# AshuiRUA/NPI-GNN

Hardware: AMD Instinct MI355X
Metric: edges/sec per GNN layer (fwd+bwd) (higher is better)
Workload: dtype f32; 1 GPU; C4 synthetic ncRNA-protein bipartite graph, N=1000000 nodes, E=20000000 directed edges (both directions, Zipf-skewed protein side), 1 SAGEConv layer 256->256 fp32, fwd+bwd incl. dX/dW/db, graph+features resident in HBM; parallelism=single GPU, hip_graph_replay=False, setup_steps=40, csr_sorted_columns=True

## Files before the change

### include/npi_gnn.h

```cpp
#ifndef NPI_GNN_H
#define NPI_GNN_H

#include <stdint.h>

#ifdef __cplusplus
extern "C" {
#endif

#define NPI_OK 0
#define NPI_ERR_ARG (-1)
#define NPI_ERR_LAUNCH (-2)
#define NPI_ERR_WORKSPACE (-3)

#ifndef NPI_ITEM_EDGES
#define NPI_ITEM_EDGES 256
#endif

#define NPI_F32 0
#define NPI_BF16 1

const char* npi_last_error(void);
int npi_abi_version(void);

int64_t npi_csr_workspace_bytes(int64_t E, int64_t N);
int64_t npi_item_edges(int64_t nnz_max);
int64_t npi_num_items(int64_t nnz_max, int64_t item_edges);

#define NPI_CSR_DROP_EQUAL 1
#define NPI_CSR_SORT_COLUMNS 2
int npi_csr_build_ex(const int64_t* key_nodes, const int64_t* val_nodes, int64_t E, int64_t N,
                     int64_t n_cols, int add_self_loops, int64_t loop_col_offset, int build_flags,
                     int32_t* rowptr, int32_t* col, int32_t* eid, int32_t* rowidx,
                     int32_t* item_row, int64_t item_edges, int32_t* status,
                     void* workspace, int64_t workspace_bytes, void* stream);

int npi_edge_positions(const int32_t* eid, const int32_t* rowptr, int64_t N, int64_t nnz_max,
                       int64_t E, int32_t* pos_of, void* stream);

int64_t npi_segsum_carry_elems(int64_t nnz_max, int64_t item_edges, int64_t F);
int npi_segsum_scales_supported(int64_t F, int dtype);
int npi_segsum_ex(const int32_t* rowptr, const int32_t* col, const int32_t* item_row, int64_t item_edges,
                   const float* w, int64_t N, int64_t nnz_max, const void* x, int64_t ldx,
                   const void* x2, int64_t split, void* out, int64_t ldo, int64_t F, int dtype, int mean,
                   const float* bias, float* carry, float* row_scales_out, void* stream);

#define NPI_HUB_MAX 128
int64_t npi_hub_plan_workspace_elems(void);
int npi_hub_plan(const int32_t* rowptr, const int32_t* col, int64_t N, int64_t n_cols, int64_t nnz_max, int64_t h_max,
                 int64_t min_degree, int64_t min_entries, int32_t* hub_rows, uint32_t* mask, int32_t* info, int32_t* workspace,
                 void* stream);
int npi_hub_light_side(const int32_t* rowptr, const int32_t* col, const int32_t* eid, const int32_t* rowidx, int64_t N,
                       int64_t nnz_max, const int32_t* hub_rows, int64_t H, int64_t nnz_max_light, int64_t item_edges,
                       int32_t* rowptr_l, int32_t* col_l, int32_t* eid_l, int32_t* rowidx_l, int32_t* item_row_l, void* stream);
int64_t npi_segsum_hub_slabs(int64_t n_cols);
int64_t npi_segsum_hub_partial_elems(int64_t n_cols);
int npi_segsum_hub(const int32_t* hub_rows, int64_t H, const uint32_t* mask, const int32_t* rowptr, int64_t N, int64_t n_cols,
                   const float* col_scale, const float* x, int64_t ldx, float* out, int64_t ldo, int64_t F, int mean,
                   float* partial, float* row_scales_out, void* stream);

int npi_row_weight_sum(const int32_t* rowptr, const float* w, int64_t N, float* deg, void* stream);
int npi_gcn_norm(const int32_t* rowidx, const int32_t* col, const int32_t* rowptr, const float* w,
                 const float* deg, const int32_t* deg_rowptr, int64_t N, int64_t nnz_max, float* norm,
                 void* stream);
int npi_entry_col_scale(const int32_t* col, const int32_t* rowptr, const float* table, const float* w_in, int64_t N, int64_t n_cols,
                        int64_t nnz_max, float* w_out, void* stream);
int npi_row_inv_count(const int32_t* rowptr, int64_t N, float* inv_cnt, void* stream);
int npi_entry_weights(const int32_t* eid, const int32_t* rowidx, const int32_t* rowptr,
                      const float* edge_w, const float* loop_w_node, float fill,
                      int64_t N, int64_t nnz_max, float* w_entry, void* stream);
int npi_edge_dot(const int32_t* rowptr, const int32_t* col, const int32_t* rowidx, const int32_t* eid, int64_t N, int64_t n_cols,
                 int64_t nnz_max, int64_t n_edges, const float* a, int64_t lda, const float* b, int64_t ldb, int64_t F,
                 const float* row_scale, const float* mul, float* g_entry, float* gm_entry, float* d_edge, float* d_loop,
                 void* stream);
int npi_gcn_norm_bwd(const int32_t* rowptr, const int32_t* col, const int32_t* rowidx, const int32_t* eid, int64_t N,
                     int64_t nnz_max, int64_t n_edges, const float* g_entry, const float* deg, const float* s_a, const float* s_b,
                     float* d_edge, float* d_loop, void* stream);
int npi_hold_cus(int workgroups, int64_t nanoseconds, uint64_t* start_word, void* stream);
int npi_relu_backward(const float* dy, int64_t ldd, const float* y, int64_t ldy, int64_t M, int64_t F, float* dz, int64_t ldz,
                      void* stream);

#define NPI_STATUS_BAD_ROW_ID 8
int npi_rows_gather(const void* x, int64_t ldx, int64_t n_src, const int64_t* idx, int64_t n, int64_t F, void* out, int64_t ldo,
                    int dtype, int32_t* status, void* stream);

int npi_l2_normalize_rows(const float* x, int64_t ldx, int64_t M, int64_t F, float eps, float* y, int64_t ldy, float* norm,
                          void* stream);
int npi_l2_normalize_rows_bwd(const float* dy, int64_t ldd, const float* y, int64_t ldy, const float* norm, int64_t M, int64_t F,
                              float eps, float* dx, int64_t ldx, void* stream);


int64_t npi_colsum_workspace_elems(int64_t M, int64_t N);
int npi_colsum(const float* X, int64_t ldx, int64_t M, int64_t N, float* out, float* workspace,
               int64_t workspace_elems, void* stream);
int64_t npi_linear_bwd_weight_workspace_elems(int64_t M, int64_t K, int64_t N);

#define NPI_GEMM_EXACT_F32 1
#define NPI_GEMM_SPLIT_BF16 2
#define NPI_GEMM_A_ZERO_PADDED 4
#define NPI_GEMM_WORKSPACE_PREPARED 8
#define NPI_GEMM_RESERVE_CUS(n) ((((n) / 8) & 0xff) << 8)
#define NPI_GEMM_RESERVED_CUS_OF(flags) ((((flags) >> 8) & 0xff) * 8)
#define NPI_GEMM_SPLIT_F16X2 16
#define NPI_PREPARE_F16X2 4
int64_t npi_linear_workspace_bytes(int64_t K, int64_t N);
int npi_row_scales(const float* A, int64_t lda, int64_t M, int64_t K, float* scales, void* stream);
int npi_linear_prepare(const void* W, int64_t ldw, int64_t K, int64_t N, int which, int dtype, void* workspace,
                       int64_t workspace_bytes, void* stream);
int npi_linear_bwd_weight_ex(const void* A, int64_t lda, const void* dC, int64_t lddc,
                             void* dW, int64_t lddw, void* db,
                             int64_t M, int64_t K, int64_t N,
                             float* workspace, int64_t workspace_elems, int dtype, int flags, int shared,
                             const float* a_col_scales, const float* dc_col_scales, void* stream);
int64_t npi_col_scales_workspace_elems(int64_t M, int64_t K);
int npi_col_scales(const float* A, int64_t lda, int64_t M, int64_t K, const float* row_scales, float* scales,
                   float* workspace, int64_t workspace_elems, void* stream);
int npi_linear_fwd_ex(const void* A, int64_t lda, const void* W, int64_t ldw, const void* bias,
                       const float* rowscale, void* C, int64_t ldc,
                       int64_t M, int64_t K, int64_t N, int relu, int dtype, int flags,
                       void* workspace, int64_t workspace_bytes, const float* a_scales, void* stream);
int npi_linear_bwd_data_ex(const void* dC, int64_t lddc, const void* W, int64_t ldw,
                            const float* rowscale, void* dA, int64_t ldda,
                            int64_t M, int64_t K, int64_t N, int dtype, int flags,
                            void* workspace, int64_t workspace_bytes, const float* dc_scales, void* stream);

int npi_linear_fwd_scores_supported(int64_t M, int64_t K, int64_t N);
int npi_linear_fwd_scores(const float* A, int64_t lda, const float* W, int64_t ldw, const float* att, float* C, int64_t ldc,
                              float* sc0, float* sc1, int64_t M, int64_t K, int64_t N, void* workspace, int64_t workspace_bytes,
                              const float* a_scales, void* stream);
int npi_linear_bwd_data_rank2_supported(int64_t M, int64_t K, int64_t N);
int npi_linear_bwd_data_rank2(const float* dC, int64_t lddc, const float* W, int64_t ldw, const float* row0,
                                  const float* row1, const float* col0, const float* col1, float* dA, int64_t ldda,
                                  int64_t M, int64_t K, int64_t N, void* workspace, int64_t workspace_bytes,
                                  const float* dc_scales, void* stream);

int npi_gat_rank2_cols(const float* W, int64_t ldw, const float* att, int64_t K, int64_t C, float* U, void* stream);
int npi_gat_rank2_tail(const float* P, const float* W, int64_t ldw, const float* att, int64_t K, int64_t C, float* dw, int64_t lddw,
                       float* datt, void* stream);

int npi_conv_fwd(const int32_t* rowptr, const int32_t* col, const int32_t* item_row, int64_t item_edges,
                 const float* w_entry, int64_t N, int64_t nnz_max, const void* x, int64_t ldx, int64_t F, int mean,
                 void* agg, int64_t ldagg, float* carry, const void* W, int64_t ldw, const void* bias, void* out,
// ... 153 lines not shown
```

### npi_gnn_amd/_lib.py

```python
from __future__ import annotations

import ctypes
import os
from ctypes import c_char_p, c_float, c_int, c_int64, c_void_p

import torch

HERE = os.path.dirname(os.path.abspath(__file__))
LIB_PATH = os.environ.get("NPI_GNN_LIB") or os.path.join(HERE, "libnpi_gnn.so")

NPI_F32 = 0
NPI_BF16 = 1
NPI_GEMM_EXACT_F32 = 1
NPI_GEMM_SPLIT_BF16 = 2
NPI_GEMM_A_ZERO_PADDED = 4
NPI_GEMM_WORKSPACE_PREPARED = 8
NPI_GEMM_SPLIT_F16X2 = 16
NPI_PREPARE_F16X2 = 4
NPI_STATUS_BAD_ROW_ID = 8
NPI_STATUS_BAD_TARGET_ID = 16
NPI_STATUS_BAD_SAMPLE_SIZES = 32
NPI_HUB_MAX = 128


def NPI_GEMM_RESERVE_CUS(n: int) -> int:
    n = int(n)
    if n < 0 or n > 128 or n % 8:
        raise ValueError(f"NPI_GEMM_RESERVE_CUS: a multiple of 8 in [0, 128], got {n}")
    return (n // 8) << 8

_P = c_void_p
_I = c_int64

PROTOTYPES = {
    "npi_last_error": (c_char_p, []),
    "npi_abi_version": (c_int, []),
    "npi_csr_workspace_bytes": (_I, [_I, _I]),
    "npi_item_edges": (_I, [_I]),
    "npi_num_items": (_I, [_I, _I]),
    "npi_csr_build_ex": (c_int, [_P, _P, _I, _I, _I, c_int, _I, c_int, _P, _P, _P, _P, _P, _I, _P, _P, _I, _P]),
    "npi_edge_positions": (c_int, [_P, _P, _I, _I, _I, _P, _P]),
    "npi_segsum_carry_elems": (_I, [_I, _I, _I]),
    "npi_segsum_ex": (c_int, [_P, _P, _P, _I, _P, _I, _I, _P, _I, _P, _I, _P, _I, _I, c_int, c_int, _P, _P, _P, _P]),
    "npi_segsum_scales_supported": (c_int, [_I, c_int]),
    "npi_hub_plan_workspace_elems": (_I, []),
    "npi_hub_plan": (c_int, [_P, _P, _I, _I, _I, _I, _I, _I, _P, _P, _P, _P, _P]),
    "npi_hub_light_side": (c_int, [_P, _P, _P, _P, _I, _I, _P, _I, _I, _I, _P, _P, _P, _P, _P, _P]),
    "npi_segsum_hub_slabs": (_I, [_I]),
    "npi_segsum_hub_partial_elems": (_I, [_I]),
    "npi_segsum_hub": (c_int, [_P, _I, _P, _P, _I, _I, _P, _P, _I, _P, _I, _I, c_int, _P, _P, _P]),
    "npi_row_weight_sum": (c_int, [_P, _P, _I, _P, _P]),
    "npi_gcn_norm": (c_int, [_P, _P, _P, _P, _P, _P, _I, _I, _P, _P]),
    "npi_row_inv_count": (c_int, [_P, _I, _P, _P]),
    "npi_entry_col_scale": (c_int, [_P, _P, _P, _P, _I, _I, _I, _P, _P]),
    "npi_entry_weights": (c_int, [_P, _P, _P, _P, _P, c_float, _I, _I, _P, _P]),
    "npi_edge_dot": (c_int, [_P, _P, _P, _P, _I, _I, _I, _I, _P, _I, _P, _I, _I, _P, _P, _P, _P, _P, _P, _P]),
    "npi_gcn_norm_bwd": (c_int, [_P, _P, _P, _P, _I, _I, _I, _P, _P, _P, _P, _P, _P, _P]),
    "npi_relu_backward": (c_int, [_P, _I, _P, _I, _I, _I, _P, _I, _P]),
    "npi_rows_gather": (c_int, [_P, _I, _I, _P, _I, _I, _P, _I, c_int, _P, _P]),
    "npi_l2_normalize_rows": (c_int, [_P, _I, _I, _I, c_float, _P, _I, _P, _P]),
    "npi_l2_normalize_rows_bwd": (c_int, [_P, _I, _P, _I, _P, _I, _I, c_float, _P, _I, _P]),
    "npi_colsum_workspace_elems": (_I, [_I, _I]),
    "npi_colsum": (c_int, [_P, _I, _I, _I, _P, _P, _I, _P]),
    "npi_linear_bwd_weight_workspace_elems": (_I, [_I, _I, _I]),
    "npi_linear_workspace_bytes": (_I, [_I, _I]),
    "npi_row_scales": (c_int, [_P, _I, _I, _I, _P, _P]),
    "npi_linear_fwd_ex": (c_int, [_P, _I, _P, _I, _P, _P, _P, _I, _I, _I, _I, c_int, c_int, c_int, _P, _I, _P, _P]),
    "npi_linear_bwd_data_ex": (c_int, [_P, _I, _P, _I, _P, _P, _I, _I, _I, _I, c_int, c_int, _P, _I, _P, _P]),
    "npi_linear_prepare": (c_int, [_P, _I, _I, _I, c_int, c_int, _P, _I, _P]),
    "npi_hold_cus": (c_int, [c_int, _I, _P, _P]),
    "npi_linear_fwd_scores_supported": (c_int, [_I, _I, _I]),
    "npi_linear_fwd_scores": (c_int, [_P, _I, _P, _I, _P, _P, _I, _P, _P, _I, _I, _I, _P, _I, _P, _P]),
    "npi_linear_bwd_data_rank2_supported": (c_int, [_I, _I, _I]),
    "npi_linear_bwd_data_rank2": (c_int, [_P, _I, _P, _I, _P, _P, _P, _P, _P, _I, _I, _I, _I, _P, _I, _P, _P]),
    "npi_gat_rank2_cols": (c_int, [_P, _I, _P, _I, _I, _P, _P]),
    "npi_gat_rank2_tail": (c_int, [_P, _P, _I, _P, _I, _I, _P, _I, _P, _P]),
    "npi_linear_bwd_weight_ex": (c_int, [_P, _I, _P, _I, _P, _I, _P, _I, _I, _I, _P, _I, c_int, c_int, c_int, _P, _P, _P]),
    "npi_col_scales_workspace_elems": (_I, [_I, _I]),
    "npi_col_scales": (c_int, [_P, _I, _I, _I, _P, _P, _P, _I, _P]),
    "npi_conv_fwd": (c_int, [_P, _P, _P, _I, _P, _I, _I, _P, _I, _I, c_int, _P, _I, _P, _P, _I, _P, _P, _I, _I, _I, c_int, c_int, c_int,
                             c_int, _P, _I, _P]),
    "npi_conv_bwd": (c_int, [_P, _I, _P, _I, _P, _I, _I, _I, _I, c_int, c_int, _P, _I, _P, _I, _P, _P, _I, _P, _I, _P, _P, _I, _P, _I,
                             c_int, _P, _P, _P, _I, _P, _I, _P, _I, _P, _P]),
    "npi_gat_aggregate_fused": (c_int, [_P, _P, _P, _P, _I, _I, _I, _P, _I, _P, _I, _P, _I, _I, _P, _P, c_float, _P, c_int, _P, _P, _P, _P,
                                            _P]),
    "npi_gat_scores": (c_int, [_P, _I, _P, _I, _I, _I, _P, _P, _P]),
    "npi_gat_aggregate_ex": (c_int, [_P, _P, _P, _I, _I, _I, _P, _I, _P, _I, _P, _I, _I, _I, _P, _P, _P, _P, c_float, c_int,
                                     _P, _P, _P, _P, _P, _P, _P, _P]),
    "npi_gat_pack_targets": (c_int, [_P, _P, _P, _P, _I, _P, _P]),
    "npi_gat_backward_fused_heads": (c_int, [_P, _P, _P, _P, _I, _I, _I, _P, _I, _P, _I, _P, _I, _P, _I, _I, _I, _P, _P, c_float, _P,
                                                 _P, _P, _P, _P, _I, _P]),
    "npi_gat_rank1_add": (c_int, [_P, _I, _P, _P, _P, _I, _I, _I, _P]),
    "npi_gat_rowdot": (c_int, [_P, _I, _P, _I, _P, _I, _I, _I, _P, _P]),
    "npi_gat_edge_grad_ex": (c_int, [_P, _P, _P, _I, _I, _P, _I, _P, _I, _P, _I, _I, _I, _P, _P, _P, _P, _P, c_float,
                                     c_int, _P, _P, _P]),
    "npi_seg_scan_workspace_elems": (_I, [_I, _I]),
    "npi_seg_rowsum_ex": (c_int, [_P, _P, _P, _P, _I, _I, _I, _P, _P, _I, _P]),
    "npi_gat_softmax_stats_ex": (c_int, [_P, _P, _P, _P, _P, _I, _I, _I, c_float, _P, _P, _P, _P, _I, _P]),
    "npi_gat_aggregate_scores": (c_int, [_P, _P, _P, _I, _I, _I, _P, _I, _P, _I, _P, _I, _I, _P, _P, _P, _P, c_int, _P, _P]),
    "npi_gat_rowdot_colsum_workspace_elems": (_I, [_I, _I, _I]),
    "npi_gat_rowdot_colsum_relu": (c_int, [_P, _I, _P, _I, _P, _I, _I, _I, _P, _P, _P, _I, _P, _I, _P]),
    "npi_entry_transpose_map": (c_int, [_P, _P, _P, _P, _P, _I, _I, _P, _P]),
    "npi_gat_att_grad_workspace_elems": (_I, [_I, _I, _I]),
    "npi_gat_att_grad": (c_int, [_P, _I, _P, _P, _I, _I, _I, _P, _P, _I, _P]),
    "npi_topk_score": (c_int, [_P, _I, _P, _I, _I, _P, _P]),
    "npi_graph_bounds": (c_int, [_P, _I, _I, _P, _P]),
    "npi_topk_select": (c_int, [_P, _P, _I, _I, c_float, _P, _P, _P, _P, _I, _P]),
    "npi_topk_sorted_workspace_bytes": (_I, [_I]),
    "npi_topk_select_sorted": (c_int, [_P, _P, _P, _I, _I, c_float, _P, _P, _P, _P, _I, _P]),
    "npi_topk_gather": (c_int, [_P, _I, _P, _P, _P, _P, _I, _I, _I, _P, _I, _P, _P, _P, _P]),
    "npi_filter_adj_workspace_elems": (_I, [_I]),
    "npi_filter_adj": (c_int, [_P, _P, _I, _P, _P, _P, _P, _P, c_int, _P]),
    "npi_filter_adj_newpos_offset": (_I, [_I]),
    "npi_csr_filter_max_rows": (_I, []),
    "npi_csr_filter_workspace_elems": (_I, [_I]),
    "npi_csr_filter": (c_int, [_P, _P, _P, _P, _P, _P, _I, _I, _P, _P, _P, _P, _P, _I, _P, _P, _P]),
    "npi_readout_max_mean": (c_int, [_P, _I, _P, _I, _I, _P, _P]),
    "npi_topk_gather_bwd": (c_int, [_P, _I, _P, _P, _P, _I, _I, _P, _I, _P, _P, _I, _P, _P, _P]),
    "npi_topk_gather_bwd_ex": (c_int, [_P, _I, _P, _P, _P, _I, _I, _P, _I, _P, _P, _I, _P, _P, _P]),
    "npi_topk_weight_grad_workspace_elems": (_I, [_I, _I]),
    "npi_topk_weight_grad": (c_int, [_P, _I, _P, _P, _P, _I, _I, _P, _P, _P, _I, _P]),
    "npi_readout_max_mean_bwd": (c_int, [_P, _I, _P, _I, _I, _P, _P, _P, _I, _P]),
    "npi_readout_max_mean_bwd_ex": (c_int, [_P, _I, _P, _I, _I, _P, _P, _P, _I, _I, _P]),
    "npi_confusion_update": (c_int, [_P, _I, _I, _P, _I, _P, _P]),
    "npi_mlp_head_fwd": (c_int, [_P, _I, _P, _I, _P, _I, _I, _I, _P, _P, _I, _P, _P, _I, _P, _P, _I, _P, c_float, c_int,
                                 _P, _P, _P, _P, _P]),
    "npi_mlp_head_workspace_elems": (_I, [_I, _I, _I, _I]),
    "npi_mlp_head_bwd": (c_int, [_I, _I, _I, _I, _I, _P, _P, _P, _P, c_float, c_int, _P, _P, _P, _P, _P, _P, _P, _P, _P, _P, _P, _P,
                                 _P, _I, _P]),
    "npi_subgraph_sizes": (c_int, [_P, _P, _P, _P, _I, _P, _P, _P, _P]),
    "npi_subgraph_fill": (c_int, [_P, _P, _P, _P, _I, _P, _P, _P, _P, _P, _P, _I, _I, _P, _P]),
    "npi_subgraph_features": (c_int, [_P, _I, _I, _P, _P, _P, _I, _I, _P, _I, _P]),
    "npi_sample_counts": (c_int, [_P, _I, _P, _I, _I, c_float, _P, _P, _P]),
# ... 67 lines not shown
```

### npi_gnn_amd/csrc/segsum_hub.hip

```cpp
#include "npi_common.h"

namespace npi {

constexpr int HUB_WAVES = 8;
constexpr int HUB_PER_WAVE = NPI_HUB_MAX / HUB_WAVES;
constexpr int HUB_THREADS = HUB_WAVES * WAVE;
constexpr int HUB_TILE = 32;
constexpr int HUB_TILE_LOADS = HUB_TILE / HUB_WAVES;
constexpr int HUB_SLAB = 2048;
constexpr int HUB_F = 256;
constexpr int HUB_MASK_WORDS = NPI_HUB_MAX / 32;
constexpr int FIN_WAVES = 16;
static_assert(HUB_PER_WAVE == 16 && HUB_MASK_WORDS == 4, "the wave's 16 mask bits are cut out of four 32-bit words");
static_assert(HUB_TILE == 32 && HUB_TILE % HUB_WAVES == 0, "one mask row per lane of a half wave");

__device__ __forceinline__ uint32_t wave_pattern(const uint4& m, int w) {
    return ((m.x >> w) & 0x01010101u) | (((m.y >> w) & 0x01010101u) << 1) | (((m.z >> w) & 0x01010101u) << 2) |
           (((m.w >> w) & 0x01010101u) << 3);
}
constexpr uint32_t pattern_bit(int k) { return 1u << (8 * (k & 3) + (k >> 2)); }
__device__ __forceinline__ int hub_of(int k, int w) { return ((k >> 2) * 32) + (k & 3) * 8 + w; }

__device__ __forceinline__ void hub_prefetch(const float* __restrict__ x, int64_t ldx, const uint4* __restrict__ mask,
                                             const float* __restrict__ col_scale, int t0, int r1, int w, int lane,
                                             float4 (&pre)[HUB_TILE_LOADS], uint32_t& pat_n, uint32_t& need_n, float& cs_n) {
    const int row = t0 + lane;
    const bool valid = lane < HUB_TILE && row < r1;
    uint4 m = make_uint4(0u, 0u, 0u, 0u);
    if (valid) m = mask[row];
    cs_n = (valid && col_scale != nullptr) ? col_scale[row] : 1.f;
    pat_n = wave_pattern(m, w);
    need_n = (uint32_t)__ballot((m.x | m.y | m.z | m.w) != 0u);
#pragma unroll
    for (int t = 0; t < HUB_TILE_LOADS; ++t) {
        const int i = w + HUB_WAVES * t;
        if ((need_n >> i) & 1u)
            pre[t] = *reinterpret_cast<const float4*>(x + (int64_t)(t0 + i) * ldx + lane * 4);
    }
}

__global__ void __launch_bounds__(HUB_THREADS, 4)
hub_stream_kernel(const float* __restrict__ x, int64_t ldx, const uint4* __restrict__ mask, const float* __restrict__ col_scale,
                  int n_cols, int H, float* __restrict__ partial) {
    __shared__ float4 tile[HUB_TILE][WAVE];
    const int lane = lane_id();
    const int w = uniform_i(threadIdx.x >> 6);
    const int r0 = blockIdx.x * HUB_SLAB;
    const int r1 = min(r0 + HUB_SLAB, n_cols);

    float4 acc[HUB_PER_WAVE];
#pragma unroll
    for (int k = 0; k < HUB_PER_WAVE; ++k) acc[k] = make_float4(0.f, 0.f, 0.f, 0.f);

    float4 pre[HUB_TILE_LOADS];
#pragma unroll
    for (int t = 0; t < HUB_TILE_LOADS; ++t) pre[t] = make_float4(0.f, 0.f, 0.f, 0.f);
    uint32_t pat_n = 0, need_n = 0;
    float cs_n = 1.f;
    if (r0 < r1) hub_prefetch(x, ldx, mask, col_scale, r0, r1, w, lane, pre, pat_n, need_n, cs_n);
    for (int t0 = r0; t0 < r1; t0 += HUB_TILE) {
        __syncthreads();
#pragma unroll
        for (int t = 0; t < HUB_TILE_LOADS; ++t) {
            const int i = w + HUB_WAVES * t;
            if ((need_n >> i) & 1u) tile[i][lane] = pre[t];
        }
        const uint32_t pat = pat_n;
        const float cs = cs_n;
        __syncthreads();
        if (t0 + HUB_TILE < r1) hub_prefetch(x, ldx, mask, col_scale, t0 + HUB_TILE, r1, w, lane, pre, pat_n, need_n, cs_n);
#pragma unroll
        for (int k = 0; k < HUB_PER_WAVE; ++k) {
            uint32_t m = (uint32_t)__ballot((pat & pattern_bit(k)) != 0u);
            while (m != 0u) {
                const int i = uniform_i(__builtin_ctz(m));
                m &= m - 1u;
                const float s = bcast_f(cs, i);
                const float4 v = tile[i][lane];
                acc[k].x = fmaf(v.x, s, acc[k].x);
                acc[k].y = fmaf(v.y, s, acc[k].y);
                acc[k].z = fmaf(v.z, s, acc[k].z);
                acc[k].w = fmaf(v.w, s, acc[k].w);
            }
        }
    }
    float4* __restrict__ dst = reinterpret_cast<float4*>(partial) + (int64_t)blockIdx.x * NPI_HUB_MAX * WAVE;
#pragma unroll
    for (int k = 0; k < HUB_PER_WAVE; ++k) {
        const int j = hub_of(k, w);
        if (j < H) dst[(int64_t)j * WAVE + lane] = acc[k];
    }
}

__device__ __forceinline__ float4 add4(const float4& a, const float4& b) { return make_float4(a.x + b.x, a.y + b.y, a.z + b.z, a.w + b.w); }

__global__ void __launch_bounds__(FIN_WAVES * WAVE)
hub_finish_kernel(const float* __restrict__ partial, int n_slabs, const int32_t* __restrict__ hub_rows, const int32_t* __restrict__ rowptr,
                  int mean, float* __restrict__ out, int64_t ldo, float* __restrict__ scale_out) {
    __shared__ float4 part[FIN_WAVES][WAVE];
    const int lane = lane_id();
    const int w = uniform_i(threadIdx.x >> 6);
    const int j = blockIdx.x;
    const int chunk = (n_slabs + FIN_WAVES - 1) / FIN_WAVES;
    const int s0 = w * chunk, s1 = min(s0 + chunk, n_slabs);
    const float4* __restrict__ src = reinterpret_cast<const float4*>(partial) + (int64_t)j * WAVE + lane;
    const int64_t step = (int64_t)NPI_HUB_MAX * WAVE;
    float4 a = make_float4(0.f, 0.f, 0.f, 0.f);
    int s = s0;
    for (; s + 8 <= s1; s += 8) {
        float4 v[8];
#pragma unroll
        for (int u = 0; u < 8; ++u) v[u] = src[(int64_t)(s + u) * step];
#pragma unroll
        for (int u = 0; u < 8; ++u) a = add4(a, v[u]);
    }
    for (; s < s1; ++s) a = add4(a, src[(int64_t)s * step]);
    part[w][lane] = a;
    __syncthreads();
    if (w != 0) return;
    a = part[0][lane];
#pragma unroll
    for (int g = 1; g < FIN_WAVES; ++g) a = add4(a, part[g][lane]);
    const int r = hub_rows[j];
    float sc = 1.f;
    if (mean) sc = 1.f / (float)max(rowptr[r + 1] - rowptr[r], 1);
    const float4 t = make_float4(fmaf(a.x, sc, 0.f), fmaf(a.y, sc, 0.f), fmaf(a.z, sc, 0.f), fmaf(a.w, sc, 0.f));
    *reinterpret_cast<float4*>(out + (int64_t)r * ldo + lane * 4) = t;
    if (scale_out != nullptr) {
        float m = fmaxf(fmaxf(fabsf(t.x), fabsf(t.y)), fmaxf(fabsf(t.z), fabsf(t.w)));
#pragma unroll
        for (int o = 32; o >= 1; o >>= 1) m = fmaxf(m, __shfl_xor(m, o));
        if (lane == 0) scale_out[r] = pow2_scale_of(m);
    }
}

}

using namespace npi;

extern "C" int64_t npi_segsum_hub_slabs(int64_t n_cols) { return n_cols <= 0 ? 0 : ceil_div(n_cols, HUB_SLAB); }

extern "C" int64_t npi_segsum_hub_partial_elems(int64_t n_cols) {
    return n_cols < 0 ? -1 : (npi_segsum_hub_slabs(n_cols) > 0 ? npi_segsum_hub_slabs(n_cols) : 1) * NPI_HUB_MAX * HUB_F;
}

extern "C" int npi_segsum_hub(const int32_t* hub_rows, int64_t H, const uint32_t* mask, const int32_t* rowptr, int64_t N, int64_t n_cols,
                              const float* col_scale, const float* x, int64_t ldx, float* out, int64_t ldo, int64_t F, int mean,
                              float* partial, float* row_scales_out, void* stream_) {
    hipStream_t stream = (hipStream_t)stream_;
    NPI_REQUIRE(H >= 0 && H <= NPI_HUB_MAX, "npi_segsum_hub: H must be in [0, NPI_HUB_MAX]");
    NPI_REQUIRE(F == HUB_F, "npi_segsum_hub: f32 rows of 256 columns only");
    NPI_REQUIRE(N >= 0 && n_cols >= 0 && n_cols < ((int64_t)1 << 31) - HUB_SLAB, "npi_segsum_hub: bad size");
    if (H == 0) return NPI_OK;
    NPI_REQUIRE(hub_rows && mask && rowptr && x && out && partial, "npi_segsum_hub: null pointer");
    NPI_REQUIRE(ldx >= F && ldo >= F && ldx % 4 == 0 && ldo % 4 == 0 && ((uintptr_t)x % 16) == 0 && ((uintptr_t)out % 16) == 0 &&
                    ((uintptr_t)partial % 16) == 0 && ((uintptr_t)mask % 16) == 0,
                "npi_segsum_hub: rows and masks must be 16-byte aligned");
    const int64_t n_slabs = npi_segsum_hub_slabs(n_cols);
    if (n_slabs > 0) {
        hipLaunchKernelGGL(hub_stream_kernel, dim3((unsigned)n_slabs), dim3(HUB_THREADS), 0, stream, x, ldx,
                           reinterpret_cast<const uint4*>(mask), col_scale, (int)n_cols, (int)H, partial);
        int rc = check_launch("npi_segsum_hub(stream)");
        if (rc != NPI_OK) return rc;
    }
    hipLaunchKernelGGL(hub_finish_kernel, dim3((unsigned)H), dim3(FIN_WAVES * WAVE), 0, stream, partial, (int)n_slabs, hub_rows, rowptr,
                       mean, out, ldo, row_scales_out);
    return check_launch("npi_segsum_hub(finish)");
}
```

### npi_gnn_amd/functional.py

```python
from __future__ import annotations

from typing import Optional

import torch

from ._lib import (NPI_BF16, NPI_F32, NPI_GEMM_A_ZERO_PADDED, NPI_GEMM_EXACT_F32, NPI_GEMM_RESERVE_CUS, NPI_GEMM_SPLIT_F16X2,
                   NPI_GEMM_WORKSPACE_PREPARED, NPI_PREPARE_F16X2, check, load, ptr, require_gpu, stream_ptr)
from .graph import BipartiteGraph, CSRGraph, CSRSide, GraphBatch, HubPlan, as_graph, note_status
from .schedule import DEFAULT, Schedule


_PROFILE = None
_PROFILE_TAGS = None


class _tag_events:

    def __init__(self, tag, dev):
        self.rec = _PROFILE_TAGS
        if self.rec is not None:
            self.tag, self.dev = tag, dev
            self.e0, self.e1 = torch.cuda.Event(enable_timing=True), torch.cuda.Event(enable_timing=True)

    def __enter__(self):
# ... 54 lines not shown
    if t.dtype not in (torch.float32, torch.bfloat16):
        raise TypeError(f"{name} must be float32 or bfloat16 (got {t.dtype})")
    if like is not None and t.dtype != like.dtype:
        raise TypeError(f"{name} is {t.dtype} but the other operand is {like.dtype}")
    return t if t.is_contiguous() else t.contiguous()


def _fcp(t: torch.Tensor, name: str) -> torch.Tensor:
    if t.dim() == 2 and t.stride(1) == 1 and t.stride(0) >= t.size(1):
        if t.dtype not in (torch.float32, torch.bfloat16):
            raise TypeError(f"{name} must be float32 or bfloat16 (got {t.dtype})")
        return t
    return _fc(t, name)


def _code(t: torch.Tensor) -> int:
    return NPI_BF16 if t.dtype == torch.bfloat16 else NPI_F32


def _check_out(out: torch.Tensor, rows: int, cols: int, like: torch.Tensor, what: str) -> None:
    if (out.dim() != 2 or out.size(0) != rows or out.size(1) != cols or out.dtype != like.dtype or out.stride(1) != 1
            or out.device != like.device):
        raise ValueError(f"{what}: out must be [{rows}, {cols}] {like.dtype} with unit column stride on {like.device} "
                         f"(got {tuple(out.shape)} {out.dtype}, strides {tuple(out.stride())}, {out.device})")


def segsum_scales_ok(side: CSRSide, x: torch.Tensor, out: Optional[torch.Tensor] = None) -> bool:
    return (x.dtype == torch.float32 and x.size(1) == 256 and side.nnz_max > 0 and x.stride(0) % 4 == 0 and x.data_ptr() % 16 == 0
            and (out is None or (out.stride(0) % 4 == 0 and out.data_ptr() % 16 == 0)))


def segsum(graph: CSRGraph, side: CSRSide, x: torch.Tensor, w: Optional[torch.Tensor] = None,
           mean: bool = False, bias: Optional[torch.Tensor] = None,
           out: Optional[torch.Tensor] = None, x2: Optional[torch.Tensor] = None,
           scales_out: Optional[torch.Tensor] = None, hub: Optional[HubPlan] = None,
           col_scale: Optional[torch.Tensor] = None) -> torch.Tensor:
    dev = require_gpu(x, w, bias, x2, col_scale)
    x = _fcp(x, "x")
    if bias is not None:
        bias = _fc(bias, "bias", x)
    N, F = side.n_rows, x.size(1)
    split = x.size(0)
    if x2 is not None:
        x2 = _fcp(x2, "x2")
        if x2.dtype != x.dtype:
            raise TypeError(f"x2 is {x2.dtype} but the other operand is {x.dtype}")
        if x2.size(1) != F:
            raise ValueError("x2 must have the width of x")
        if x2.stride(0) != x.stride(0):
            x2 = x2.contiguous()
            if x2.stride(0) != x.stride(0):
                x = x.contiguous()
    if side.n_cols > split + (x2.size(0) if x2 is not None else 0):
        raise ValueError(f"the table has {split + (x2.size(0) if x2 is not None else 0)} rows, the adjacency indexes {side.n_cols}")
    if out is None:
        out = torch.empty((N, F), dtype=x.dtype, device=dev)
    else:
        _check_out(out, N, F, x, "segsum")
    full = side
    if hub is not None:
        if not (x.dtype == torch.float32 and F == 256 and x2 is None and bias is None and x.stride(0) % 4 == 0 and x.data_ptr() % 16 == 0
                and out.stride(0) % 4 == 0 and out.data_ptr() % 16 == 0 and hub.light.n_rows == N):
            raise ValueError("segsum(hub=): the streaming path takes one f32 table of 256 columns, 16-byte aligned rows, no bias")
        if col_scale is not None:
            col_scale = _f32c(col_scale, "col_scale")
            if col_scale.numel() != side.n_cols:
                raise ValueError(f"segsum: col_scale has {col_scale.numel()} elements, the table {side.n_cols} rows")
        side = hub.light
    elif col_scale is not None:
        raise ValueError("segsum: col_scale belongs to the streaming path (hub=); the plain launch takes per-entry weights")
    carry = side.carry(F)
    prof = _PROFILE
    if prof is not None:
        ev0, ev1 = torch.cuda.Event(enable_timing=True), torch.cuda.Event(enable_timing=True)
        ev0.record(torch.cuda.current_stream(dev))
    if scales_out is not None and (scales_out.dtype != torch.float32 or scales_out.numel() != N or not scales_out.is_contiguous()):
        raise ValueError("segsum: scales_out must be a contiguous float32 vector with one element per output row")
    check(load().npi_segsum_ex(ptr(side.rowptr), ptr(side.col), ptr(side.item_row), side.item, ptr(w), N, side.nnz_max,
                                ptr(x), x.stride(0), ptr(x2), split if x2 is not None else 0, ptr(out), out.stride(0), F,
                                _code(x), 1 if mean else 0, ptr(bias), ptr(carry), ptr(scales_out), stream_ptr(dev)), "npi_segsum")
    if hub is not None:
        check(load().npi_segsum_hub(ptr(hub.hub_rows), hub.H, ptr(hub.mask), ptr(full.rowptr), N, full.n_cols, ptr(col_scale), ptr(x),
                                    x.stride(0), ptr(out), out.stride(0), F, 1 if mean else 0, ptr(hub.partial()), ptr(scales_out),
                                    stream_ptr(dev)), "npi_segsum_hub")
    if prof is not None:
        ev1.record(torch.cuda.current_stream(dev))
        prof.append((ev0, ev1))
    return out


def hub_plan_for(graph: CSRGraph, side: CSRSide, x: torch.Tensor, out: Optional[torch.Tensor] = None) -> Optional[HubPlan]:
    if not graph.hub_stream or not segsum_scales_ok(side, x, out) or x.size(0) != side.n_cols:
        return None
    return side.hub_plan()




def _gflags(sch: Schedule) -> int:
    return NPI_GEMM_EXACT_F32 if sch.gemm_exact_f32 else 0


def _f16x2(sch: Schedule, rows: int, K: int, N: int, dtype) -> bool:
    return (sch.f16x2_min_rows is not None and not sch.gemm_exact_f32 and rows >= sch.f16x2_min_rows and dtype == torch.float32
            and f16x2_shape(rows, K, N))


def _gemm_workspace(K: int, N: int, dev) -> torch.Tensor:
    return torch.empty(int(load().npi_linear_workspace_bytes(K, N)), dtype=torch.uint8, device=dev)


def _pad128(k: int) -> int:
    return (int(k) + 127) // 128 * 128


def padded_aggregate_buffer(x: torch.Tensor, K: int, rows: int, bf16_ok: bool = False):
    if (x.dtype not in ((torch.float32, torch.bfloat16) if bf16_ok else (torch.float32,)) or x.size(1) != K or K % 128 == 0
            or 2 * _pad128(K) > 3 * K or rows < 128):
        return None
    return torch.zeros((rows, _pad128(K)), dtype=x.dtype, device=x.device)


def f16x2_shape(M: int, K: int, N: int) -> bool:
    return M >= 128 and K % 32 == 0 and N % 128 == 0


def _check_scales(scales: Optional[torch.Tensor], rows: int, what: str) -> None:
    if scales is not None and (scales.dtype != torch.float32 or scales.dim() != 1 or scales.numel() != rows or not scales.is_contiguous()):
        raise ValueError(f"{what}: the row scales must be a contiguous float32 vector with one element per row ({rows}), "
                         f"got {tuple(scales.shape)} {scales.dtype}")


def row_scales(a: torch.Tensor) -> torch.Tensor:
    dev = require_gpu(a)
    if a.dtype != torch.float32 or a.dim() != 2 or a.stride(1) != 1:
        raise TypeError("row_scales: a float32 matrix with unit column stride")
    out = torch.empty(a.size(0), dtype=torch.float32, device=dev)
    check(load().npi_row_scales(ptr(a), a.stride(0), a.size(0), a.size(1), ptr(out), stream_ptr(dev)), "npi_row_scales")
    return out


class Planes:
    __slots__ = ("buf", "f16")

    def __init__(self, buf: torch.Tensor, f16: bool = False):
        self.buf, self.f16 = buf, bool(f16)


def _planes_for(ws: Optional["Planes"], f16: bool, what: str) -> torch.Tensor:
    if not isinstance(ws, Planes):
        raise TypeError(f"{what}: ws must come from prepare_weight (a functional.Planes)")
    if ws.f16 != f16:
        raise ValueError(f"{what}: the prepared weight copy holds {'fp16 x 2' if ws.f16 else 'bf16 x 3'} planes, this call runs on "
                         f"{'fp16 x 2 (row scales given)' if f16 else 'bf16 x 3 (no row scales)'}: prepare_weight(..., f16={f16})")
    return ws.buf


def prepare_weight(weight: torch.Tensor, backward: bool = True, f16: bool = False):
    K, N = weight.shape
    if (weight.dtype not in (torch.float32, torch.bfloat16) or K % 32 or N % 32 or weight.stride(1) != 1
            or not weight.is_cuda or (f16 and weight.dtype != torch.float32)):
        return None, None
    lib = load()
    dev = weight.device
    one = int(lib.npi_linear_workspace_bytes(K, N))
    ws = torch.empty(one * (2 if backward else 1), dtype=torch.uint8, device=dev)
    check(lib.npi_linear_prepare(ptr(weight), weight.stride(0), K, N, (3 if backward else 1) | (NPI_PREPARE_F16X2 if f16 else 0),
# ... 1581 lines not shown
```

### npi_gnn_amd/graph.py

```python
from __future__ import annotations

from dataclasses import dataclass, field
from typing import Dict, Optional

import torch

from . import _lib
from ._lib import check, load, ptr, require_gpu, stream_ptr

_DEBUG = False

_PENDING = []
_PENDING_MAX = 256


def set_debug(flag: bool) -> None:
    global _DEBUG
    _DEBUG = bool(flag)


def pending_status(device=None) -> list:
    if device is None:
        out = list(_PENDING)
        _PENDING.clear()
        return out
    out = [t for t in _PENDING if t.device == device]
    _PENDING[:] = [t for t in _PENDING if t.device != device]
    return out


def raise_on_status(values) -> None:
    if any(int(v) & 1 for v in values):
        raise IndexError("edge_index holds a node id outside [0, num_nodes): the edges were dropped by the graph build "
                         "(PyG's index_select / scatter raise here)")
    if any(int(v) & _lib.NPI_STATUS_BAD_ROW_ID for v in values):
        raise IndexError("res_n_id holds a row id outside [0, N_src): the row was gathered as zeros (npi_rows_gather; torch's "
                         "index_select raises here)")
    if any(int(v) & _lib.NPI_STATUS_BAD_TARGET_ID for v in values):
        raise IndexError("NeighborSampler: a target id outside [0, num_nodes): it was dropped (no entry sampled for it; "
                         "npi_sample_counts)")
    if any(int(v) & _lib.NPI_STATUS_BAD_SAMPLE_SIZES for v in values):
        raise ValueError("npi_sample_select / npi_sample_relabel: the offsets or counts they were given belong to another call; "
                         "the entries concerned were not written")
    if any(int(v) & 4 for v in values):
        raise ValueError("InteractionGraph.batch: the n_nodes / n_pairs it was given do not belong to its keys (the device counted "
                         "other totals); that batch holds placeholders only (node 0 / graph 0 rows, padding edges, zero features).  "
                         "Totals must come from sizes() of the same keys")


def note_status(status: torch.Tensor) -> None:
    if torch.cuda.is_current_stream_capturing():
        return
    if _DEBUG:
        raise_on_status([status.item()])
        return
    _PENDING.append(status)
    if len(_PENDING) > _PENDING_MAX:
        check_pending()


def check_pending() -> None:
    st = pending_status()
    if st:
        by_dev = {}
        for t in st:
            by_dev.setdefault(t.device, []).append(t)
        for ts in by_dev.values():
            raise_on_status(torch.cat(ts).tolist())


CARRY_SLOTS = 6


@dataclass
class CSRSide:
    rowptr: torch.Tensor
    col: torch.Tensor
    eid: torch.Tensor
    rowidx: torch.Tensor
    item_row: torch.Tensor
    status: torch.Tensor
    nnz_max: int
    n_items: int
    _inv_cnt: Optional[torch.Tensor] = None
    _carry: Dict[tuple, torch.Tensor] = field(default_factory=dict)
    n_rows: int = -1
    n_cols: int = -1
    item: int = 0
    _hub: Optional["HubPlan"] = None
    _hub_asked: bool = False
    rect_hub: bool = False

    def inv_count(self) -> torch.Tensor:
        if self._inv_cnt is None:
            dev = self.rowptr.device
            out = torch.empty(self.n_rows, dtype=torch.float32, device=dev)
            check(load().npi_row_inv_count(ptr(self.rowptr), self.n_rows, ptr(out), stream_ptr(dev)),
                  "npi_row_inv_count")
            self._inv_cnt = out
        return self._inv_cnt

    def hub_plan(self) -> Optional["HubPlan"]:
        if not self._hub_asked:
            if (self.n_rows != self.n_cols and not self.rect_hub) or self.n_cols < HUB_MIN_COLS or self.nnz_max <= 0:
                self._hub_asked = True
            elif not torch.cuda.is_current_stream_capturing():
                self._hub = build_hub_plan(self)
                self._hub_asked = True
        return self._hub

    def carry(self, F: int) -> torch.Tensor:
        dev = self.rowptr.device
        key = (F, _lib.stream_ptr(dev))
        buf = self._carry.pop(key, None)
        if buf is None:
            n = int(load().npi_segsum_carry_elems(self.nnz_max, self.item, F))
            buf = torch.zeros(n, dtype=torch.float32, device=dev)
            if len(self._carry) >= CARRY_SLOTS and not torch.cuda.is_current_stream_capturing():
                self._carry.pop(next(iter(self._carry)))
        elif _DEBUG and not torch.cuda.is_current_stream_capturing():
            self._check_counters(buf)
        self._carry[key] = buf
        return buf

    def _check_counters(self, buf: torch.Tensor) -> None:
        n_wg = -(-self.n_items // 4)
        n = n_wg + 2 * (-(-n_wg // 64))
        if n and int(buf[:n].view(torch.int32).abs().max()) != 0:
            raise _lib.NpiError("aggregation scratch: an arrival counter is not zero between launches -- two launches shared the "
                                "buffer concurrently or one was aborted; call reset_carry() on this side")

    def reset_carry(self) -> None:
        self._carry.clear()


HUB_MIN_COLS = 262_144
HUB_DEGREE_DIV = 512
HUB_ENTRIES_PER_STREAMED_ROW = 2


@dataclass
class HubPlan:
    H: int
    n_entries: int
    hub_rows: torch.Tensor
    mask: torch.Tensor
    light: CSRSide
    _partial: Dict[int, torch.Tensor] = field(default_factory=dict)

    def partial(self) -> torch.Tensor:
        dev = self.mask.device
        key = _lib.stream_ptr(dev)
        buf = self._partial.pop(key, None)
        if buf is None:
            buf = torch.empty(int(load().npi_segsum_hub_partial_elems(self.mask.size(0))), dtype=torch.float32, device=dev)
            if len(self._partial) >= CARRY_SLOTS and not torch.cuda.is_current_stream_capturing():
                self._partial.pop(next(iter(self._partial)))
        self._partial[key] = buf
        return buf


def build_hub_plan(side: CSRSide, h_max: int = _lib.NPI_HUB_MAX, min_degree: Optional[int] = None,
                   min_entries: Optional[int] = None) -> Optional[HubPlan]:
    if side.n_rows != side.n_cols and not side.rect_hub:
        raise ValueError("build_hub_plan: one-table sides with n_cols == n_rows, or the sides of a BipartiteGraph, only")
    lib = load()
    dev = side.rowptr.device
    N = side.n_rows
    if N <= 0 or side.nnz_max <= 0:
        return None
    if min_degree is None:
        min_degree = max(-(-side.n_cols // HUB_DEGREE_DIV), 2)
    if min_entries is None:
        min_entries = HUB_ENTRIES_PER_STREAMED_ROW * side.n_cols
    i32 = dict(dtype=torch.int32, device=dev)
    hub_rows = torch.empty(_lib.NPI_HUB_MAX, **i32)
    mask = torch.empty((side.n_cols, _lib.NPI_HUB_MAX // 32), **i32)
    info = torch.empty(4, **i32)
    ws = torch.empty(int(lib.npi_hub_plan_workspace_elems()), **i32)
    s = stream_ptr(dev)
    check(lib.npi_hub_plan(ptr(side.rowptr), ptr(side.col), N, side.n_cols, side.nnz_max, int(h_max), int(min_degree), int(min_entries),
                           ptr(hub_rows), ptr(mask), ptr(info), ptr(ws), s), "npi_hub_plan")
    H, n_entries = info.tolist()[:2]
    if H == 0:
        return None
    nnz_max = side.nnz_max - n_entries
    n_items = int(lib.npi_num_items(nnz_max, side.item))
    rowptr = torch.empty(N + 1, **i32)
    col = torch.empty(max(nnz_max, 1), **i32)
    eid = torch.empty(max(nnz_max, 1), **i32)
    rowidx = torch.empty(max(nnz_max, 1), **i32)
    item_row = torch.empty(n_items + 1, **i32)
    check(lib.npi_hub_light_side(ptr(side.rowptr), ptr(side.col), ptr(side.eid), ptr(side.rowidx), N, side.nnz_max, ptr(hub_rows), H,
                                 nnz_max, side.item, ptr(rowptr), ptr(col), ptr(eid), ptr(rowidx), ptr(item_row), s),
          "npi_hub_light_side")
    light = CSRSide(rowptr, col, eid, rowidx, item_row, side.status, nnz_max, n_items)
    light.n_rows, light.n_cols, light.item, light.rect_hub = N, side.n_cols, side.item, side.rect_hub
    light._hub_asked = True
    return HubPlan(H, n_entries, hub_rows, mask, light)


def item_hint(nnz_max: int) -> int:
    return int(load().npi_item_edges(int(nnz_max)))


def build_side(key: torch.Tensor, val: torch.Tensor, n_rows: int, n_cols: int, self_loops: bool = True,
               loop_col_offset: int = 0, drop_equal: bool = True, item: Optional[int] = None,
               sort_columns: bool = False) -> CSRSide:
    lib = load()
    dev = require_gpu(key, val)
    E, N = int(key.numel()), int(n_rows)
    nnz_max = E + (N if self_loops else 0)
    item = item_hint(nnz_max) if item is None else int(item)
    n_items = int(lib.npi_num_items(nnz_max, item))
    if n_items < 0:
        raise ValueError(f"build_side: item must be 64 or 256 (got {item})")
    i32 = dict(dtype=torch.int32, device=dev)
    rowptr = torch.empty(N + 1, **i32)
    col = torch.empty(max(nnz_max, 1), **i32)
    eid = torch.empty(max(nnz_max, 1), **i32)
    rowidx = torch.empty(max(nnz_max, 1), **i32)
    item_row = torch.empty(n_items + 1, **i32)
    status = torch.empty(1, **i32)
    ws_bytes = int(lib.npi_csr_workspace_bytes(E, N))
    ws = torch.empty(ws_bytes, dtype=torch.uint8, device=dev)
    check(lib.npi_csr_build_ex(ptr(key), ptr(val), E, N, int(n_cols), 1 if self_loops else 0,
                               int(loop_col_offset), (1 if drop_equal else 0) | (2 if sort_columns else 0), ptr(rowptr), ptr(col), ptr(eid),
                               ptr(rowidx), ptr(item_row), item, ptr(status), ptr(ws), ws_bytes, stream_ptr(dev)),
          "npi_csr_build_ex")
    note_status(status)
    side = CSRSide(rowptr, col, eid, rowidx, item_row, status, nnz_max, n_items)
    side.n_rows, side.n_cols, side.item = N, int(n_cols), item
    return side


class CSRGraph:

    def __init__(self, edge_index: torch.Tensor, num_nodes: int, self_loops: bool = True, by_dst: Optional[CSRSide] = None,
                 symmetric: bool = False, item: Optional[int] = None, sort_columns: bool = False, keep_equal: bool = False,
                 hub_stream: bool = True):
        if edge_index.dtype != torch.int64 or edge_index.dim() != 2 or edge_index.size(0) != 2:
            raise ValueError("edge_index must be a LongTensor of shape [2, E]")
        require_gpu(edge_index)
        self.num_nodes = int(num_nodes)
        self.num_edges = int(edge_index.size(1))
        self.self_loops = bool(self_loops)
        self.device = edge_index.device
        self._ei_version = edge_index._version
        self._ei_ptr = edge_index.data_ptr()
        self.symmetric = bool(symmetric)
        self._src = edge_index[0].contiguous()
        self._dst = edge_index[1].contiguous()
        self._item = item if by_dst is None else by_dst.item
        self.sort_columns = bool(sort_columns)
        self.keep_equal = bool(keep_equal)
        self.hub_stream = bool(hub_stream)
        if self.keep_equal and self.self_loops:
            raise ValueError("CSRGraph: keep_equal=True (existing self loops stay ordinary entries) needs self_loops=False")
        self.by_dst = by_dst if by_dst is not None else \
            build_side(self._dst, self._src, self.num_nodes, self.num_nodes, self.self_loops, drop_equal=not self.keep_equal,
                       item=self._item, sort_columns=self.sort_columns)
        self._by_src: Optional[CSRSide] = None

    @property
    def by_src(self) -> CSRSide:
        if self._by_src is None:
            self._by_src = build_side(self._src, self._dst, self.num_nodes, self.num_nodes, self.self_loops,
                                      drop_equal=not self.keep_equal, item=self.by_dst.item, sort_columns=self.sort_columns)
        return self._by_src

    def built_from(self, edge_index: torch.Tensor, num_nodes: Optional[int] = None) -> bool:
        return (self.num_edges == edge_index.size(1) and self._ei_version == edge_index._version
                and self._ei_ptr == edge_index.data_ptr() and (num_nodes is None or self.num_nodes == int(num_nodes)))

    def inv_count(self, side: CSRSide) -> torch.Tensor:
        return side.inv_count()

    def carry(self, side: CSRSide, F: int) -> torch.Tensor:
        return side.carry(F)

    def nnz(self) -> int:
        n = int(self.by_dst.rowptr[-1].item())
# ... 209 lines not shown
```

Before: 3.645 billion edges/s.

## Balance hub rows across waves and batch hub tile accumulations

Adds a host-built slot table that gives each wave of the hub streaming kernel hubs chosen greedily by degree, so hub work spreads evenly across waves instead of following a fixed interleaved mapping. Each tile's mask bits are transposed through shared-memory ballots into per-hub words, replacing the per-hub pattern-extraction ballot. The inner accumulation loop is unrolled to issue up to four tile loads before the FMAs to raise memory-level parallelism. This adds extra ballots, a double-buffered shared words array, and one host sync at plan build time.

```diff
diff --git a/include/npi_gnn.h b/include/npi_gnn.h
--- a/include/npi_gnn.h
+++ b/include/npi_gnn.h
@@ -45,6 +45,8 @@
                    const float* bias, float* carry, float* row_scales_out, void* stream);
 
 #define NPI_HUB_MAX 128
+#define NPI_HUB_WAVES 8
+#define NPI_HUB_SLOTS 16
 int64_t npi_hub_plan_workspace_elems(void);
 int npi_hub_plan(const int32_t* rowptr, const int32_t* col, int64_t N, int64_t n_cols, int64_t nnz_max, int64_t h_max,
                  int64_t min_degree, int64_t min_entries, int32_t* hub_rows, uint32_t* mask, int32_t* info, int32_t* workspace,
@@ -56,7 +58,7 @@
 int64_t npi_segsum_hub_partial_elems(int64_t n_cols);
 int npi_segsum_hub(const int32_t* hub_rows, int64_t H, const uint32_t* mask, const int32_t* rowptr, int64_t N, int64_t n_cols,
                    const float* col_scale, const float* x, int64_t ldx, float* out, int64_t ldo, int64_t F, int mean,
-                   float* partial, float* row_scales_out, void* stream);
+                   float* partial, float* row_scales_out, const int32_t* slot_hub, void* stream);
 
 int npi_row_weight_sum(const int32_t* rowptr, const float* w, int64_t N, float* deg, void* stream);
 int npi_gcn_norm(const int32_t* rowidx, const int32_t* col, const int32_t* rowptr, const float* w,
diff --git a/npi_gnn_amd/_lib.py b/npi_gnn_amd/_lib.py
--- a/npi_gnn_amd/_lib.py
+++ b/npi_gnn_amd/_lib.py
@@ -21,6 +21,8 @@
 NPI_STATUS_BAD_TARGET_ID = 16
 NPI_STATUS_BAD_SAMPLE_SIZES = 32
 NPI_HUB_MAX = 128
+NPI_HUB_WAVES = 8
+NPI_HUB_SLOTS = 16
 
 
 def NPI_GEMM_RESERVE_CUS(n: int) -> int:
@@ -48,7 +50,7 @@
     "npi_hub_light_side": (c_int, [_P, _P, _P, _P, _I, _I, _P, _I, _I, _I, _P, _P, _P, _P, _P, _P]),
     "npi_segsum_hub_slabs": (_I, [_I]),
     "npi_segsum_hub_partial_elems": (_I, [_I]),
-    "npi_segsum_hub": (c_int, [_P, _I, _P, _P, _I, _I, _P, _P, _I, _P, _I, _I, c_int, _P, _P, _P]),
+    "npi_segsum_hub": (c_int, [_P, _I, _P, _P, _I, _I, _P, _P, _I, _P, _I, _I, c_int, _P, _P, _P, _P]),
     "npi_row_weight_sum": (c_int, [_P, _P, _I, _P, _P]),
     "npi_gcn_norm": (c_int, [_P, _P, _P, _P, _P, _P, _I, _I, _P, _P]),
     "npi_row_inv_count": (c_int, [_P, _I, _P, _P]),
diff --git a/npi_gnn_amd/csrc/segsum_hub.hip b/npi_gnn_amd/csrc/segsum_hub.hip
--- a/npi_gnn_amd/csrc/segsum_hub.hip
+++ b/npi_gnn_amd/csrc/segsum_hub.hip
@@ -2,8 +2,8 @@
 
 namespace npi {
 
-constexpr int HUB_WAVES = 8;
-constexpr int HUB_PER_WAVE = NPI_HUB_MAX / HUB_WAVES;
+constexpr int HUB_WAVES = NPI_HUB_WAVES;
+constexpr int HUB_PER_WAVE = NPI_HUB_SLOTS;
 constexpr int HUB_THREADS = HUB_WAVES * WAVE;
 constexpr int HUB_TILE = 32;
 constexpr int HUB_TILE_LOADS = HUB_TILE / HUB_WAVES;
@@ -11,26 +11,56 @@
 constexpr int HUB_F = 256;
 constexpr int HUB_MASK_WORDS = NPI_HUB_MAX / 32;
 constexpr int FIN_WAVES = 16;
-static_assert(HUB_PER_WAVE == 16 && HUB_MASK_WORDS == 4, "the wave's 16 mask bits are cut out of four 32-bit words");
+constexpr int HUB_ADD_AHEAD = 4;
+static_assert(HUB_WAVES * HUB_PER_WAVE == NPI_HUB_MAX && HUB_MASK_WORDS == 4 && 32 % HUB_PER_WAVE == 0,
+              "every hub has a slot; a mask row is one uint4; the hubs a wave transposes lie in one mask word");
 static_assert(HUB_TILE == 32 && HUB_TILE % HUB_WAVES == 0, "one mask row per lane of a half wave");
 
-__device__ __forceinline__ uint32_t wave_pattern(const uint4& m, int w) {
-    return ((m.x >> w) & 0x01010101u) | (((m.y >> w) & 0x01010101u) << 1) | (((m.z >> w) & 0x01010101u) << 2) |
-           (((m.w >> w) & 0x01010101u) << 3);
-}
-constexpr uint32_t pattern_bit(int k) { return 1u << (8 * (k & 3) + (k >> 2)); }
-__device__ __forceinline__ int hub_of(int k, int w) { return ((k >> 2) * 32) + (k & 3) * 8 + w; }
+__device__ __forceinline__ int hub_of_lane(const int32_t* __restrict__ slot_hub, int w, int lane, int H) {
+    int j = -1;
+    if (lane < HUB_PER_WAVE) j = slot_hub != nullptr ? slot_hub[w * HUB_PER_WAVE + lane] : lane * HUB_WAVES + w;
+    return (j >= 0 && j < H) ? j : -1;
+}
+
+template <int N>
+__device__ __forceinline__ void hub_add(float4& a, uint32_t& m, float cs, const float4 (*tile)[WAVE], int lane) {
+    int i[N];
+    float4 v[N];
+#pragma unroll
+    for (int u = 0; u < N; ++u) {
+        i[u] = uniform_i(__builtin_ctz(m));
+        m &= m - 1u;
+        v[u] = tile[i[u]][lane];
+    }
+#pragma unroll
+    for (int u = 0; u < N; ++u) {
+        const float s = bcast_f(cs, i[u]);
+        a.x = fmaf(v[u].x, s, a.x);
+        a.y = fmaf(v[u].y, s, a.y);
+        a.z = fmaf(v[u].z, s, a.z);
+        a.w = fmaf(v[u].w, s, a.w);
+    }
+}
 
 __device__ __forceinline__ void hub_prefetch(const float* __restrict__ x, int64_t ldx, const uint4* __restrict__ mask,
                                              const float* __restrict__ col_scale, int t0, int r1, int w, int lane,
-                                             float4 (&pre)[HUB_TILE_LOADS], uint32_t& pat_n, uint32_t& need_n, float& cs_n) {
+                                             float4 (&pre)[HUB_TILE_LOADS], uint32_t* __restrict__ words, uint32_t& need_n, float& cs_n) {
     const int row = t0 + lane;
     const bool valid = lane < HUB_TILE && row < r1;
     uint4 m = make_uint4(0u, 0u, 0u, 0u);
     if (valid) m = mask[row];
     cs_n = (valid && col_scale != nullptr) ? col_scale[row] : 1.f;
-    pat_n = wave_pattern(m, w);
     need_n = (uint32_t)__ballot((m.x | m.y | m.z | m.w) != 0u);
+    const int q = (w * HUB_PER_WAVE) >> 5;
+    const uint32_t mw = (q == 0 ? m.x : (q == 1 ? m.y : (q == 2 ? m.z : m.w))) >> ((w * HUB_PER_WAVE) & 31);
+    uint32_t rows[HUB_PER_WAVE];
+#pragma unroll
+    for (int k = 0; k < HUB_PER_WAVE; ++k) rows[k] = (uint32_t)__ballot((mw & (1u << k)) != 0u);
+    if (lane == 0) {
+#pragma unroll
+        for (int k = 0; k < HUB_PER_WAVE; k += 4)
+            *reinterpret_cast<uint4*>(words + w * HUB_PER_WAVE + k) = make_uint4(rows[k], rows[k + 1], rows[k + 2], rows[k + 3]);
+    }
 #pragma unroll
     for (int t = 0; t < HUB_TILE_LOADS; ++t) {
         const int i = w + HUB_WAVES * t;
@@ -41,13 +71,15 @@
 
 __global__ void __launch_bounds__(HUB_THREADS, 4)
 hub_stream_kernel(const float* __restrict__ x, int64_t ldx, const uint4* __restrict__ mask, const float* __restrict__ col_scale,
-                  int n_cols, int H, float* __restrict__ partial) {
+                  const int32_t* __restrict__ slot_hub, int n_cols, int H, float* __restrict__ partial) {
     __shared__ float4 tile[HUB_TILE][WAVE];
+    __shared__ __align__(16) uint32_t words[2][NPI_HUB_MAX];
     const int lane = lane_id();
     const int w = uniform_i(threadIdx.x >> 6);
     const int r0 = blockIdx.x * HUB_SLAB;
     const int r1 = min(r0 + HUB_SLAB, n_cols);
 
+    const int my_hub = hub_of_lane(slot_hub, w, lane, H);
     float4 acc[HUB_PER_WAVE];
 #pragma unroll
     for (int k = 0; k < HUB_PER_WAVE; ++k) acc[k] = make_float4(0.f, 0.f, 0.f, 0.f);
@@ -55,9 +87,10 @@
     float4 pre[HUB_TILE_LOADS];
 #pragma unroll
     for (int t = 0; t < HUB_TILE_LOADS; ++t) pre[t] = make_float4(0.f, 0.f, 0.f, 0.f);
-    uint32_t pat_n = 0, need_n = 0;
+    uint32_t need_n = 0;
+    int buf = 0;
     float cs_n = 1.f;
-    if (r0 < r1) hub_prefetch(x, ldx, mask, col_scale, r0, r1, w, lane, pre, pat_n, need_n, cs_n);
+    if (r0 < r1) hub_prefetch(x, ldx, mask, col_scale, r0, r1, w, lane, pre, words[0], need_n, cs_n);
     for (int t0 = r0; t0 < r1; t0 += HUB_TILE) {
         __syncthreads();
 #pragma unroll
@@ -65,30 +98,28 @@
             const int i = w + HUB_WAVES * t;
             if ((need_n >> i) & 1u) tile[i][lane] = pre[t];
         }
-        const uint32_t pat = pat_n;
         const float cs = cs_n;
         __syncthreads();
-        if (t0 + HUB_TILE < r1) hub_prefetch(x, ldx, mask, col_scale, t0 + HUB_TILE, r1, w, lane, pre, pat_n, need_n, cs_n);
+        const uint32_t mine = my_hub >= 0 ? words[buf][my_hub] : 0u;
+        if (t0 + HUB_TILE < r1) hub_prefetch(x, ldx, mask, col_scale, t0 + HUB_TILE, r1, w, lane, pre, words[buf ^ 1], need_n, cs_n);
 #pragma unroll
         for (int k = 0; k < HUB_PER_WAVE; ++k) {
-            uint32_t m = (uint32_t)__ballot((pat & pattern_bit(k)) != 0u);
+            uint32_t m = (uint32_t)bcast_i((int)mine, k);
             while (m != 0u) {
-                const int i = uniform_i(__builtin_ctz(m));
-                m &= m - 1u;
-                const float s = bcast_f(cs, i);
-                const float4 v = tile[i][lane];
-                acc[k].x = fmaf(v.x, s, acc[k].x);
-                acc[k].y = fmaf(v.y, s, acc[k].y);
-                acc[k].z = fmaf(v.z, s, acc[k].z);
-                acc[k].w = fmaf(v.w, s, acc[k].w);
+                const int n = __builtin_popcount(m);
+                if (n >= HUB_ADD_AHEAD) hub_add<HUB_ADD_AHEAD>(acc[k], m, cs, tile, lane);
+                else if (n == 3) hub_add<3>(acc[k], m, cs, tile, lane);
+                else if (n == 2) hub_add<2>(acc[k], m, cs, tile, lane);
+                else hub_add<1>(acc[k], m, cs, tile, lane);
             }
         }
+        buf ^= 1;
     }
     float4* __restrict__ dst = reinterpret_cast<float4*>(partial) + (int64_t)blockIdx.x * NPI_HUB_MAX * WAVE;
 #pragma unroll
     for (int k = 0; k < HUB_PER_WAVE; ++k) {
-        const int j = hub_of(k, w);
-        if (j < H) dst[(int64_t)j * WAVE + lane] = acc[k];
+        const int j = bcast_i(my_hub, k);
+        if (j >= 0) dst[(int64_t)j * WAVE + lane] = acc[k];
     }
 }
 
@@ -146,7 +177,7 @@
 
 extern "C" int npi_segsum_hub(const int32_t* hub_rows, int64_t H, const uint32_t* mask, const int32_t* rowptr, int64_t N, int64_t n_cols,
                               const float* col_scale, const float* x, int64_t ldx, float* out, int64_t ldo, int64_t F, int mean,
-                              float* partial, float* row_scales_out, void* stream_) {
+                              float* partial, float* row_scales_out, const int32_t* slot_hub, void* stream_) {
     hipStream_t stream = (hipStream_t)stream_;
     NPI_REQUIRE(H >= 0 && H <= NPI_HUB_MAX, "npi_segsum_hub: H must be in [0, NPI_HUB_MAX]");
     NPI_REQUIRE(F == HUB_F, "npi_segsum_hub: f32 rows of 256 columns only");
@@ -159,7 +190,7 @@
     const int64_t n_slabs = npi_segsum_hub_slabs(n_cols);
     if (n_slabs > 0) {
         hipLaunchKernelGGL(hub_stream_kernel, dim3((unsigned)n_slabs), dim3(HUB_THREADS), 0, stream, x, ldx,
-                           reinterpret_cast<const uint4*>(mask), col_scale, (int)n_cols, (int)H, partial);
+                           reinterpret_cast<const uint4*>(mask), col_scale, slot_hub, (int)n_cols, (int)H, partial);
         int rc = check_launch("npi_segsum_hub(stream)");
         if (rc != NPI_OK) return rc;
     }
diff --git a/npi_gnn_amd/functional.py b/npi_gnn_amd/functional.py
--- a/npi_gnn_amd/functional.py
+++ b/npi_gnn_amd/functional.py
@@ -160,7 +160,7 @@
     if hub is not None:
         check(load().npi_segsum_hub(ptr(hub.hub_rows), hub.H, ptr(hub.mask), ptr(full.rowptr), N, full.n_cols, ptr(col_scale), ptr(x),
                                     x.stride(0), ptr(out), out.stride(0), F, 1 if mean else 0, ptr(hub.partial()), ptr(scales_out),
-                                    stream_ptr(dev)), "npi_segsum_hub")
+                                    ptr(hub.slot_hub), stream_ptr(dev)), "npi_segsum_hub")
     if prof is not None:
         ev1.record(torch.cuda.current_stream(dev))
         prof.append((ev0, ev1))
diff --git a/npi_gnn_amd/graph.py b/npi_gnn_amd/graph.py
--- a/npi_gnn_amd/graph.py
+++ b/npi_gnn_amd/graph.py
@@ -1,7 +1,7 @@
 from __future__ import annotations
 
 from dataclasses import dataclass, field
-from typing import Dict, Optional
+from typing import Dict, List, Optional, Sequence
 
 import torch
 
@@ -146,6 +146,7 @@
     hub_rows: torch.Tensor
     mask: torch.Tensor
     light: CSRSide
+    slot_hub: Optional[torch.Tensor] = None
     _partial: Dict[int, torch.Tensor] = field(default_factory=dict)
 
     def partial(self) -> torch.Tensor:
@@ -158,6 +159,18 @@
                 self._partial.pop(next(iter(self._partial)))
         self._partial[key] = buf
         return buf
+
+
+def balanced_hub_slots(degrees: Sequence[int], waves: int = _lib.NPI_HUB_WAVES, slots: int = _lib.NPI_HUB_SLOTS) -> List[List[int]]:
+    if len(degrees) > waves * slots:
+        raise ValueError(f"balanced_hub_slots: {len(degrees)} hubs for {waves} waves of {slots} slots")
+    table: List[List[int]] = [[] for _ in range(waves)]
+    load_of = [0] * waves
+    for j, d in enumerate(degrees):
+        w = min((w for w in range(waves) if len(table[w]) < slots), key=lambda w: (load_of[w], w))
+        table[w].append(j)
+        load_of[w] += int(d)
+    return [t + [-1] * (slots - len(t)) for t in table]
 
 
 def build_hub_plan(side: CSRSide, h_max: int = _lib.NPI_HUB_MAX, min_degree: Optional[int] = None,
@@ -197,7 +210,9 @@
     light = CSRSide(rowptr, col, eid, rowidx, item_row, side.status, nnz_max, n_items)
     light.n_rows, light.n_cols, light.item, light.rect_hub = N, side.n_cols, side.item, side.rect_hub
     light._hub_asked = True
-    return HubPlan(H, n_entries, hub_rows, mask, light)
+    rows = hub_rows[:H].long()
+    slot_hub = torch.tensor(balanced_hub_slots((side.rowptr[rows + 1] - side.rowptr[rows]).tolist()), **i32)
+    return HubPlan(H, n_entries, hub_rows, mask, light, slot_hub)
 
 
 def item_hint(nnz_max: int) -> int:
```

After: 3.560 billion edges/s. 2.3% lower.
